# qiaobeibei/PPO-RL-Satellite

Measured on NVIDIA B200. Metric: rk4_env_steps_per_sec, higher is better.
Workload: dtype f64

## Files before the change

### ppo-rl-satellite_b200/build.py

```python
from __future__ import annotations

import os
import subprocess
import sys
from concurrent.futures import ThreadPoolExecutor

HERE = os.path.dirname(os.path.abspath(__file__))
CSRC = os.path.join(HERE, "csrc")
OBJ = os.path.join(HERE, "build")
LIBDIR = os.path.join(HERE, "lib")
LIB = os.path.join(LIBDIR, "libsatb200.so")

ARCH = ["-gencode", "arch=compute_100a,code=sm_100a"]
COMMON = ["-O3", "-lineinfo", "-std=c++17", "-Xcompiler", "-fPIC"]
UNITS = {
    "rk4.cu": ["-fmad=false"],
    "env_step.cu": ["-fmad=false"],
    "gae.cu": ["-fmad=false"],
    "cw_ode.cu": ["-fmad=false"],
    "reach.cu": ["-fmad=false"],
    "actor.cu": [],
    "actor_tc.cu": [],
    "ppo_update.cu": [],
    "ppo_fb_tc.cu": [],
    "ppo_wgrad2_tc.cu": [],
    "capi.cu": [],
}


def _nvcc() -> str:
    for cand in (os.environ.get("NVCC"), "/usr/local/cuda/bin/nvcc", "nvcc"):
        if cand and (os.path.isabs(cand) and os.path.exists(cand) or not os.path.isabs(cand)):
            return cand
    return "nvcc"


def _stale(target: str, deps) -> bool:
    if not os.path.exists(target):
        return True
    t = os.path.getmtime(target)
    return any(os.path.getmtime(d) > t for d in deps)


def build(force: bool = False, verbose: bool = False) -> str:
    os.makedirs(OBJ, exist_ok=True)
    os.makedirs(LIBDIR, exist_ok=True)
    headers = [os.path.join(CSRC, f) for f in os.listdir(CSRC) if f.endswith((".cuh", ".h"))]
    headers.append(os.path.join(os.path.dirname(HERE), "include", "satb200.h"))
    nvcc = _nvcc()
    jobs = []
    objs = []
    for src, extra in UNITS.items():
        s = os.path.join(CSRC, src)
        o = os.path.join(OBJ, src.replace(".cu", ".o"))
        objs.append(o)
        if force or _stale(o, [s] + headers):
            defs = [f"-D{d}" for d in os.environ.get("SAT_NVCC_DEFINES", "").split() if d]
            cmd = [nvcc] + ARCH + COMMON + extra + defs + (["-Xptxas", "-v"] if verbose else []) + ["-c", s, "-o", o]
            jobs.append(cmd)

    def run(cmd):
        r = subprocess.run(cmd, capture_output=True, text=True)
        if r.returncode != 0:
            raise RuntimeError("nvcc failed: %s\n%s\n%s" % (" ".join(cmd), r.stdout, r.stderr))
        if verbose:
            sys.stderr.write(r.stderr)

    with ThreadPoolExecutor(max_workers=min(5, max(1, len(jobs)))) as ex:
        list(ex.map(run, jobs))
    if force or jobs or _stale(LIB, objs):
        run([nvcc] + ARCH + ["-shared", "-o", LIB] + objs + ["-Xcompiler", "-fPIC"])
    return LIB


if __name__ == "__main__":
    print(build(force="--force" in sys.argv, verbose="-v" in sys.argv))
```

### ppo-rl-satellite_b200/csrc/env_step.cu

```cuda
#include "sat_math.cuh"
#include "../../include/satb200.h"
#include <cmath>

namespace {

using namespace sat;

constexpr int kBlock = 128;
constexpr int kEnvsPerBlock = kBlock / 2;
constexpr int kFrontBlock = 64;
#ifndef SAT_FINISH_MINB
#define SAT_FINISH_MINB 7
#endif
constexpr int kFinishMinBlocks = SAT_FINISH_MINB;
constexpr int kObs = 18;
constexpr int kStatDims = 19;
constexpr int kWsHeader = 256;

SAT_DEV double shfl1(double v) { return __shfl_xor_sync(0xffffffffu, v, 1); }
SAT_DEV int shfl1(int v) { return __shfl_xor_sync(0xffffffffu, v, 1); }

SAT_DEV double clip16(double a) { return a < -1.6 ? -1.6 : (a > 1.6 ? 1.6 : a); }

__host__ __device__ inline int64_t ws_disprev_offset() { return kWsHeader; }
__host__ __device__ inline int64_t ws_partials_offset(int64_t n) { return kWsHeader + ((n * 8 + 255) / 256) * 256; }

struct Lane {
    double r[3], v[3];
    double a[3];
    double fuel_own;
    double dis_prev;
};

template <typename ActT>
SAT_DEV void load_and_gate(const SatEnvState& st, const SatEnvParams& p, const ActT* __restrict__ pa,
                           const ActT* __restrict__ ea, int64_t e, int craft, Lane& L, bool do_impulse,
                           const ActT* raw = nullptr ) {
    const int64_t ld = st.ld;
    const double* __restrict__ S = st.state;
    const int32_t* __restrict__ I = st.istate;
    const int base = craft * 6;
#pragma unroll
    for (int k = 0; k < 3; ++k) { L.r[k] = S[(base + k) * ld + e]; L.v[k] = S[(base + 3 + k) * ld + e]; }
    L.fuel_own = S[(SAT_COL_FUEL_C + craft) * ld + e];
    const double dis_stale = S[SAT_COL_DIS * ld + e];
    const int dz_stale = I[SAT_ICOL_DZ * ld + e];
    const int int_state = I[SAT_ICOL_INTSTATE * ld + e];
    {
        const ActT* act = craft ? ea : pa;
#pragma unroll
        for (int k = 0; k < 3; ++k) L.a[k] = clip16((double)(raw ? raw[k] : act[e * 3 + k]));
    }
    bool frozen;
    if (p.flag != 1) frozen = (craft == 0) && (dis_stale < p.d_range) && (dz_stale != 0);
    else frozen = (craft == 1) && (dz_stale == 0);
    if (frozen) { L.a[0] = 0.0; L.a[1] = 0.0; L.a[2] = 0.0; }
    if (!do_impulse) return;
    double d[3];
#pragma unroll
    for (int k = 0; k < 3; ++k) {
        const double o = shfl1(L.r[k]);
        d[k] = craft == 0 ? __dsub_rn(L.r[k], o) : __dsub_rn(o, L.r[k]);
    }
    L.dis_prev = norm3(d);
#pragma unroll
    for (int k = 0; k < 3; ++k) {
        const double s = __dadd_rn(L.v[k], L.a[k]);
        L.v[k] = int_state ? trunc(s) : s;
    }
    L.fuel_own = __dsub_rn(L.fuel_own, __dadd_rn(__dadd_rn(fabs(L.a[0]), fabs(L.a[1])), fabs(L.a[2])));
}

SAT_DEV void propagate_cw(const SatEnvParams& p, Lane& L) {
    const double x6[6] = {L.r[0], L.r[1], L.r[2], L.v[0], L.v[1], L.v[2]};
    double y6[6];
#pragma unroll
    for (int i = 0; i < 6; ++i) y6[i] = gemv6_row(p.stm + 6 * i, x6);
#pragma unroll
    for (int k = 0; k < 3; ++k) { L.r[k] = y6[k]; L.v[k] = y6[3 + k]; }
}

SAT_DEV void propagate_rk4(const SatEnvParams& p, Lane& L) {
    double X[3], V[3];
#pragma unroll
    for (int k = 0; k < 3; ++k) { X[k] = p.r_cw[k] + L.r[k]; V[k] = p.v_cw[k] + L.v[k]; }
    const Rk4Consts c = make_rk4_consts(p.h, p.mu, p.re, p.j2);
    if (p.j2 != 0.0) {
#pragma unroll 1
        for (int s = 0; s < p.substeps; ++s) rk4_step<true>(X, V, c);
    } else {
#pragma unroll 1
        for (int s = 0; s < p.substeps; ++s) rk4_step<false>(X, V, c);
    }
#pragma unroll
    for (int k = 0; k < 3; ++k) { L.r[k] = X[k] - p.r_cw[k]; L.v[k] = V[k] - p.v_cw[k]; }
}

template <typename ActT, bool OBS>
__global__ void __launch_bounds__(kFrontBlock, 14)
env_front_rk4_kernel(const SatEnvState st, const ActT* __restrict__ pa, const ActT* __restrict__ ea,
                     double* __restrict__ dis_prev_out, float* __restrict__ obs_early,
                     float* __restrict__ pa_copy, float* __restrict__ ea_copy, const __grid_constant__ SatEnvParams p) {
    const int64_t tid = (int64_t)blockIdx.x * kFrontBlock + threadIdx.x;
    const int64_t env_raw = tid >> 1;
    const int craft = (int)(tid & 1);
    const bool valid = env_raw < st.n;
    const int64_t e = valid ? env_raw : st.n - 1;
    Lane L;
    if (OBS) {
        ActT raw[3];
        const ActT* act = craft ? ea : pa;
#pragma unroll
        for (int k = 0; k < 3; ++k) raw[k] = act[e * 3 + k];
        if (valid) {
            float* dc = craft ? ea_copy : pa_copy;
#pragma unroll
            for (int k = 0; k < 3; ++k) dc[e * 3 + k] = (float)raw[k];
        }
        load_and_gate(st, p, pa, ea, e, craft, L, true, raw);
    } else {
        load_and_gate(st, p, pa, ea, e, craft, L, true);
    }
    propagate_rk4(p, L);
    if (valid) {
        const int64_t ld = st.ld;
        const int base = craft * 6;
#pragma unroll
        for (int k = 0; k < 3; ++k) { st.state[(base + k) * ld + e] = L.r[k]; st.state[(base + 3 + k) * ld + e] = L.v[k]; }
        st.state[(SAT_COL_FUEL_C + craft) * ld + e] = L.fuel_own;
        if (craft == 0) dis_prev_out[e] = L.dis_prev;
    }
    if (OBS) {
        double P[3], Pv[3], E[3], Ev[3], d[3];
#pragma unroll
        for (int k = 0; k < 3; ++k) {
            const double o_r = shfl1(L.r[k]), o_v = shfl1(L.v[k]);
            P[k] = craft == 0 ? L.r[k] : o_r;  Pv[k] = craft == 0 ? L.v[k] : o_v;
            E[k] = craft == 0 ? o_r : L.r[k];  Ev[k] = craft == 0 ? o_v : L.v[k];
            d[k] = __dsub_rn(P[k], E[k]);
        }
        const double dis = norm3(d);
        const int count_new = st.istate[SAT_ICOL_COUNT * st.ld + e] + 1;
        const bool done = (dis <= p.d_capture) || (count_new >= p.max_episode_steps);
        if (done && p.auto_reset) {
#pragma unroll
            for (int k = 0; k < 3; ++k) { P[k] = p.reset_p[k]; E[k] = p.reset_e[k]; Pv[k] = 0.0; Ev[k] = 0.0; }
        }
        if (valid) {
            float* o = obs_early + e * kObs + craft * 9;
            if (craft == 0) {
#pragma unroll
                for (int k = 0; k < 3; ++k) { o[k] = (float)__dsub_rn(P[k], E[k]); o[3 + k] = (float)__dsub_rn(Pv[k], Ev[k]); o[6 + k] = (float)P[k]; }
            } else {
#pragma unroll
                for (int k = 0; k < 3; ++k) { o[k] = (float)Pv[k]; o[3 + k] = (float)E[k]; o[6 + k] = (float)Ev[k]; }
            }
        }
    }
}

struct SolveQueue {
    double A[2 * kBlock], sth[2 * kBlock], dvm[2 * kBlock], alpha[2 * kBlock];
    int guess[2 * kBlock];
    double trig[2][4];
    int count, next;
};

template <bool EXACT = true>
SAT_DEV void queue_init(SolveQueue& q) {
    if (threadIdx.x == 0) { q.count = 0; q.next = 0; }
    if (threadIdx.x < 4) {
        const int j = threadIdx.x >> 1, k = threadIdx.x & 1;
        const double x0 = dz_guess(j);
        const double h = 1.4901161193847656e-08 * fabs(x0);
        const double2 sc = Lm<EXACT>::sincos(k ? x0 + h : x0);
        q.trig[j][2 * k] = sc.x; q.trig[j][2 * k + 1] = sc.y;
    }
    __syncthreads();
}

SAT_DEV void queue_push(SolveQueue& q, const DzNode& nd, int& slot0, int& slot1, double& alpha0, double& alpha1) {
    slot0 = -1; slot1 = -1; alpha0 = dz_guess(0); alpha1 = dz_guess(1);
    if (nd.status == 2) {
        const bool g0 = dz_degenerate(nd.A0, nd.sth, nd.dvm), g1 = dz_degenerate(nd.A1, nd.sth, nd.dvm);
        const int cnt = (g0 ? 0 : 1) + (g1 ? 0 : 1);
        if (cnt) {
            int s = atomicAdd(&q.count, cnt);
            if (!g0) { slot0 = s; q.A[s] = nd.A0; q.sth[s] = nd.sth; q.dvm[s] = nd.dvm; q.guess[s] = 0; ++s; }
            if (!g1) { slot1 = s; q.A[s] = nd.A1; q.sth[s] = nd.sth; q.dvm[s] = nd.dvm; q.guess[s] = 1; }
        }
    }
    __syncthreads();
}

#ifndef SAT_SOLVE_WARPS
#define SAT_SOLVE_WARPS 4
#endif
template <bool EXACT = true>
SAT_DEV void queue_run(SolveQueue& q) {
    const int total = q.count;
    int task = -1;
    Hybrd1<PFaiT<EXACT>> hs;
    if ((threadIdx.x >> 5) < SAT_SOLVE_WARPS)
    for (;;) {
        if (task < 0) {
            const int t = atomicAdd(&q.next, 1);
            if (t < total) {
                task = t;
                PFaiT<EXACT> f; f.A = q.A[t]; f.sth = q.sth[t]; f.dvm = q.dvm[t];
                hs.init_warm(f, dz_guess(q.guess[t]), q.trig[q.guess[t]]);
            } else task = total;
        }
        const bool active = task < total;
        if (!__any_sync(0xffffffffu, active)) break;
        if (active && hs.step()) { q.alpha[task] = hs.x; task = -1; }
    }
    __syncthreads();
}

template <bool FUSED, typename ActT, int MINB, bool EXACT>
__global__ void __launch_bounds__(kBlock, MINB)
env_step_kernel(const SatEnvState st, const ActT* __restrict__ pa, const ActT* __restrict__ ea,
                const int32_t* __restrict__ count_override, float* __restrict__ obs_f32,
                double* __restrict__ obs_f64, double* __restrict__ term_obs_f64,
                double* __restrict__ reward_out, uint8_t* __restrict__ done_out,
                const double* __restrict__ dis_prev_in, double* __restrict__ partials,
                unsigned int* __restrict__ ticket, const __grid_constant__ SatEnvParams p) {
    union SharedBlock { SolveQueue queue; double tile_term[kEnvsPerBlock][kObs]; __device__ SharedBlock() {} };
    __shared__ SharedBlock shm;
    __shared__ double tile[kEnvsPerBlock][kStatDims];
    SolveQueue& queue = shm.queue;
    double (&tile_term)[kEnvsPerBlock][kObs] = shm.tile_term;
    queue_init<EXACT>(queue);

    const int64_t tid = (int64_t)blockIdx.x * kBlock + threadIdx.x;
    const int64_t env_raw = tid >> 1;
    const int craft = (int)(tid & 1);
    const bool valid = env_raw < st.n;
    const int64_t e = valid ? env_raw : st.n - 1;
    const int64_t ld = st.ld;
    double* __restrict__ S = st.state;
    int32_t* __restrict__ I = st.istate;
    if (ticket && blockIdx.x == 0 && threadIdx.x == 0) *ticket = 0u;

    Lane L;
    load_and_gate(st, p, pa, ea, e, craft, L, FUSED);
    if (FUSED) propagate_cw(p, L);
    else L.dis_prev = dis_prev_in[e];
    const int dz_stale = I[SAT_ICOL_DZ * ld + e];
    const int count = I[SAT_ICOL_COUNT * ld + e];
    int err = I[SAT_ICOL_ERR * ld + e];
    const double ret = S[SAT_COL_RET * ld + e];

    double P[3], Pv[3], E[3], Ev[3], d[3];
#pragma unroll
    for (int k = 0; k < 3; ++k) {
        const double o_r = shfl1(L.r[k]), o_v = shfl1(L.v[k]);
        P[k] = craft == 0 ? L.r[k] : o_r;  Pv[k] = craft == 0 ? L.v[k] : o_v;
        E[k] = craft == 0 ? o_r : L.r[k];  Ev[k] = craft == 0 ? o_v : L.v[k];
        d[k] = __dsub_rn(P[k], E[k]);
    }
    const double dis = norm3(d);
    const int count_new = count_override ? count_override[e] : count + 1;
    const bool captured = dis <= p.d_capture;
    const bool timeout = count_new >= p.max_episode_steps;
    const bool done = captured || timeout;
    const double fuel_oth = shfl1(L.fuel_own);
    const double fuel_c = craft == 0 ? L.fuel_own : fuel_oth;
    double pa_gated[3];
#pragma unroll
    for (int k = 0; k < 3; ++k) { const double o = shfl1(L.a[k]); pa_gated[k] = craft == 0 ? L.a[k] : o; }

    const int le = threadIdx.x >> 1;
    const bool reset_now = done && p.auto_reset;
    const int64_t env0 = (int64_t)blockIdx.x * kEnvsPerBlock;
    const int64_t rem = st.n - env0;
    const int rows = (int)(rem < kEnvsPerBlock ? rem : kEnvsPerBlock);
    {
        double Po[3], Pvo[3], Eo[3], Evo[3];
#pragma unroll
        for (int k = 0; k < 3; ++k) {
            Po[k] = reset_now ? p.reset_p[k] : P[k];  Pvo[k] = reset_now ? 0.0 : Pv[k];
            Eo[k] = reset_now ? p.reset_e[k] : E[k];  Evo[k] = reset_now ? 0.0 : Ev[k];
        }
        if (craft == 0) {
#pragma unroll
            for (int k = 0; k < 3; ++k) { tile[le][k] = __dsub_rn(Po[k], Eo[k]); tile[le][3 + k] = __dsub_rn(Pvo[k], Evo[k]); tile[le][6 + k] = Po[k]; }
        } else {
#pragma unroll
            for (int k = 0; k < 3; ++k) { tile[le][9 + k] = Pvo[k]; tile[le][12 + k] = Eo[k]; tile[le][15 + k] = Evo[k]; }
        }
        __syncthreads();
        const int total = rows * kObs;
        for (int idx = threadIdx.x; idx < total; idx += kBlock) {
            const int row = idx / kObs, col = idx - row * kObs;
            const double val = tile[row][col];
            if (obs_f32) obs_f32[env0 * kObs + idx] = (float)val;
            if (obs_f64) obs_f64[env0 * kObs + idx] = val;
        }
    }

    const bool need_dz = !done && !p.skip_danger_zone && p.flag != 2;
    DzNode nd;
    {
        double Ri[3], Vi[3];
#pragma unroll
        for (int k = 0; k < 3; ++k) { Ri[k] = __dadd_rn(p.r_cw[k], L.r[k]); Vi[k] = __dadd_rn(p.v_cw[k], L.v[k]); }
        dz_prepare<EXACT>(craft, need_dz, Ri, Vi, fuel_c, p.u_grav, nd);
    }
    int slot0, slot1;
    double alpha0, alpha1;
    queue_push(queue, nd, slot0, slot1, alpha0, alpha1);
    queue_run<EXACT>(queue);
    if (slot0 >= 0) alpha0 = queue.alpha[slot0];
    if (slot1 >= 0) alpha1 = queue.alpha[slot1];
    __syncthreads();
    const int dz_eval = dz_finalize<EXACT>(need_dz, nd, alpha0, alpha1, nullptr);
    int dz_new = dz_stale;
    if (need_dz) {
        if (dz_eval >= 0) dz_new = dz_eval;
        else { dz_new = 0; err = 1; }
    }

    double reward = 0.0, cos_a = 0.0, cos_b = 0.0;
    if (p.flag == 2) reward = 0.0;
    else if (captured) reward = (p.flag == 0) ? 100.0 : -150.0;
    else if (timeout) reward = (p.flag == 0) ? 0.0 : 100.0;
    else {
        const bool pv4_on = pa_gated[0] != 0.0 && pa_gated[1] != 0.0 && pa_gated[2] != 0.0;
        double u1[3], w1[3], u2[3], w2[3];
#pragma unroll
        for (int k = 0; k < 3; ++k) {
            u1[k] = craft == 0 ? P[k] : d[k];   w1[k] = craft == 0 ? E[k] : Pv[k];
            u2[k] = craft == 0 ? Pv[k] : d[k];  w2[k] = craft == 0 ? Ev[k] : (pv4_on ? pa_gated[k] : Pv[k]);
        }
// ... 1 lines not shown
        double cb = cosine3(u2, w2);
        if (craft == 1) cb = pv4_on ? -cb : 0.0;
        cos_a = ca; cos_b = cb;
    }
    const double oth_a = shfl1(cos_a), oth_b = shfl1(cos_b);
    if (!captured && !timeout && p.flag != 2) {
        const double pv1 = craft == 0 ? cos_a : oth_a, pv2 = craft == 0 ? cos_b : oth_b;
        const double pv3 = craft == 0 ? oth_a : cos_a, pv4 = craft == 0 ? oth_b : cos_b;
        const double ra = (dis < L.dis_prev) ? 1.0 : -1.0;
        const double rb = (p.d_capture <= dis && dis <= 4.0 * p.d_capture) ? -1.0 : -2.0;
        const double rc = (dz_new == 0) ? -1.0 : dz_new * 0.5;
        double rr = __dadd_rn(__dadd_rn(ra, rb), rc);
        rr = __dadd_rn(rr, pv1);
        rr = __dadd_rn(rr, __dmul_rn(0.6, pv2));
        rr = __dadd_rn(rr, __dmul_rn(0.2, pv3));
        rr = __dadd_rn(rr, __dmul_rn(2.0, pv4));
        reward = (p.flag == 0) ? rr : -rr;
    }
    const double ret_new = __dadd_rn(__dmul_rn(p.gamma, ret), reward);

    if (term_obs_f64) {
        if (craft == 0) {
#pragma unroll
            for (int k = 0; k < 3; ++k) { tile_term[le][k] = d[k]; tile_term[le][3 + k] = __dsub_rn(Pv[k], Ev[k]); tile_term[le][6 + k] = P[k]; }
        } else {
#pragma unroll
            for (int k = 0; k < 3; ++k) { tile_term[le][9 + k] = Pv[k]; tile_term[le][12 + k] = E[k]; tile_term[le][15 + k] = Ev[k]; }
        }
    }

    int int_state_new = 0, count_store = count_new;
    if (reset_now) {
#pragma unroll
        for (int k = 0; k < 3; ++k) {
            P[k] = p.reset_p[k]; E[k] = p.reset_e[k]; Pv[k] = 0.0; Ev[k] = 0.0;
            L.r[k] = craft == 0 ? P[k] : E[k]; L.v[k] = 0.0;
        }
        int_state_new = 1; count_store = 0;
    }

    if (valid) {
        const int base = craft * 6;
        if (FUSED || reset_now) {
#pragma unroll
            for (int k = 0; k < 3; ++k) { S[(base + k) * ld + e] = L.r[k]; S[(base + 3 + k) * ld + e] = L.v[k]; }
        }
        if (FUSED) S[(SAT_COL_FUEL_C + craft) * ld + e] = L.fuel_own;
        if (craft == 0) {
            S[SAT_COL_DIS * ld + e] = dis;
            S[SAT_COL_RET * ld + e] = done ? 0.0 : ret_new;
            I[SAT_ICOL_DZ * ld + e] = dz_new;
            I[SAT_ICOL_COUNT * ld + e] = count_store;
            reward_out[e] = reward;
            done_out[e] = done ? 1 : 0;
        } else {
            I[SAT_ICOL_INTSTATE * ld + e] = int_state_new;
            I[SAT_ICOL_ERR * ld + e] = err;
        }
    }

    if (craft == 0) tile[le][18] = ret_new;
    __syncthreads();
    if (term_obs_f64) {
        const int total = rows * kObs;
        for (int idx = threadIdx.x; idx < total; idx += kBlock) {
            const int row = idx / kObs, col = idx - row * kObs;
            term_obs_f64[env0 * kObs + idx] = tile_term[row][col];
        }
    }
    if (partials && threadIdx.x < kStatDims) {
        const int dim = threadIdx.x;
        double sum = 0.0;
        for (int row = 0; row < rows; ++row) sum += tile[row][dim];
        const double mean = sum / rows;
        double m2 = 0.0;
        for (int row = 0; row < rows; ++row) { double t = tile[row][dim] - mean; m2 += t * t; }
        partials[((int64_t)blockIdx.x * kStatDims + dim) * 2 + 0] = mean;
        partials[((int64_t)blockIdx.x * kStatDims + dim) * 2 + 1] = m2;
    }
}

__global__ void __launch_bounds__(kBlock)
danger_zone_kernel(const double* __restrict__ rv, const double* __restrict__ dv, int64_t n, double u_grav,
                   int32_t* __restrict__ count_out, double* __restrict__ debug_out) {
    __shared__ SolveQueue queue;
    queue_init(queue);
    const int64_t tid = (int64_t)blockIdx.x * kBlock + threadIdx.x;
    const int64_t env_raw = tid >> 1;
    const int craft = (int)(tid & 1);
    const bool valid = env_raw < n;
    const int64_t e = valid ? env_raw : n - 1;
    double Ri[3], Vi[3];
#pragma unroll
    for (int k = 0; k < 3; ++k) { Ri[k] = rv[e * 12 + craft * 6 + k]; Vi[k] = rv[e * 12 + craft * 6 + 3 + k]; }
    DzNode nd;
    dz_prepare(craft, true, Ri, Vi, dv[e], u_grav, nd);
    int slot0, slot1;
    double alpha0, alpha1;
    queue_push(queue, nd, slot0, slot1, alpha0, alpha1);
    queue_run(queue);
    if (slot0 >= 0) alpha0 = queue.alpha[slot0];
    if (slot1 >= 0) alpha1 = queue.alpha[slot1];
    DzDebug dbg = {0, 0, 0, 0, 0, 0, 0, 0};
    const int dz = dz_finalize(true, nd, alpha0, alpha1, debug_out ? &dbg : nullptr);
    if (valid) {
        if (craft == 0) count_out[e] = dz;
        if (debug_out) {
            double* o = debug_out + (e * 2 + craft) * 8;
            o[0] = dbg.rf_max; o[1] = dbg.rf_min; o[2] = dbg.r_ft; o[3] = dbg.alpha0; o[4] = dbg.alpha1;
            o[5] = dbg.theta; o[6] = dbg.dvm; o[7] = dbg.f_cx;
        }
    }
}

__global__ void __launch_bounds__(kBlock)
fsolve_pfai_kernel(const double* __restrict__ dvm, const double* __restrict__ theta, const double* __restrict__ v1x,
                   const double* __restrict__ v1y, const double* __restrict__ h, const double* __restrict__ guess,
                   int64_t n, double u_grav, double* __restrict__ root_out, int32_t* __restrict__ nfev_out) {
    const int64_t i = (int64_t)blockIdx.x * kBlock + threadIdx.x;
    if (i >= n) return;
    double sth, cth;
    glibm::sincos(theta[i], &sth, &cth);
    PFai f;
    f.A = (2.0 * u_grav * (1.0 - cth)) / (h[i] * v1y[i]) - v1x[i] * sth / v1y[i];
    f.sth = sth;
    f.dvm = dvm[i];
    Hybrd1<PFai> hs;
    hs.init(f, guess[i]);
    while (!hs.step()) {}
    root_out[i] = hs.x;
    if (nfev_out) nfev_out[i] = hs.nfev;
}

__global__ void __launch_bounds__(256)
libm_eval_kernel(int fn, const double* __restrict__ x, double* __restrict__ y, int64_t n) {
    const int64_t i = (int64_t)blockIdx.x * 256 + threadIdx.x;
    if (i >= n) return;
    const double v = x[i];
    double r = 0.0, s, c;
    switch (fn) {
        case SAT_LIBM_SIN: r = glibm::sin(v); break;
        case SAT_LIBM_COS: r = glibm::cos(v); break;
        case SAT_LIBM_ACOS: r = glibm::acos(v); break;
        case SAT_LIBM_ATAN: r = glibm::atan(v); break;
        case SAT_LIBM_POW2: r = glibm::pow2(v); break;
        case SAT_LIBM_SINCOS_S: glibm::sincos(v, &s, &c); r = s; break;
        default: glibm::sincos(v, &s, &c); r = c; break;
    }
    y[i] = r;
}

struct Moments { double n, mean, m2; };
SAT_DEV Moments chan(Moments A, Moments B) {
    if (B.n == 0.0) return A;
    if (A.n == 0.0) return B;
    Moments C;
    C.n = A.n + B.n;
    const double delta = B.mean - A.mean;
    C.mean = A.mean + delta * (B.n / C.n);
    C.m2 = A.m2 + B.m2 + delta * delta * (A.n * B.n / C.n);
    return C;
}

SAT_DEV void fold_into_running(double* stats, int dim, int d, Moments B, double* std_out) {
    const double n_old = stats[0];
    const double mean_old = stats[1 + d], S_old = stats[1 + dim + d];
    double n_new, mean_new, S_new, std_new;
    if (B.n == 1.0) {
        const double x = B.mean;
        n_new = n_old + 1.0;
        if (n_new == 1.0) { mean_new = x; S_new = S_old; std_new = x; }
        else {
            mean_new = mean_old + (x - mean_old) / n_new;
            S_new = S_old + (x - mean_old) * (x - mean_new);
            std_new = sqrt(S_new / n_new);
        }
    } else {
        Moments A = {n_old, mean_old, S_old};
        Moments C = chan(A, B);
        n_new = C.n; mean_new = C.mean; S_new = C.m2;
        std_new = sqrt(S_new / n_new);
    }
    stats[1 + d] = mean_new; stats[1 + dim + d] = S_new; stats[1 + 2 * dim + d] = std_new;
    if (std_out) *std_out = std_new;
}

constexpr int kMergeThreads = 256;

SAT_DEV double block_sum_fixed(double v, double* sm) {
#pragma unroll
    for (int off = 16; off > 0; off >>= 1) v += __shfl_xor_sync(0xffffffffu, v, off);
    __syncthreads();
    if ((threadIdx.x & 31) == 0) sm[threadIdx.x >> 5] = v;
    __syncthreads();
    double t = 0.0;
#pragma unroll
    for (int w = 0; w < kMergeThreads / 32; ++w) t += sm[w];
    return t;
}

__global__ void __launch_bounds__(kMergeThreads)
stats_merge_kernel(const double* __restrict__ partials, int64_t nblocks, int64_t n_rows, int rows_per_block,
                   int ndims_in_partials, double* obs_stats, int obs_dim, double* ret_stats, double* ret_std_out,
                   unsigned int* ticket) {
    __shared__ double sm[kMergeThreads / 32];
    const int dim = blockIdx.x;
    const double N = (double)n_rows;
    double wsum = 0.0;
    for (int64_t b = threadIdx.x; b < nblocks; b += kMergeThreads) {
        const int64_t rem = n_rows - b * rows_per_block;
        const double nb = (double)(rem < rows_per_block ? rem : rows_per_block);
        wsum += nb * partials[(b * ndims_in_partials + dim) * 2 + 0];
    }
    const double grand = block_sum_fixed(wsum, sm) / N;
    double m2 = 0.0;
    for (int64_t b = threadIdx.x; b < nblocks; b += kMergeThreads) {
        const int64_t rem = n_rows - b * rows_per_block;
        const double nb = (double)(rem < rows_per_block ? rem : rows_per_block);
        const double dm = partials[(b * ndims_in_partials + dim) * 2 + 0] - grand;
        m2 += partials[(b * ndims_in_partials + dim) * 2 + 1] + nb * dm * dm;
    }
    m2 = block_sum_fixed(m2, sm);
    if (threadIdx.x == 0) {
        Moments B = {N, grand, m2};
        if (dim < obs_dim) { if (obs_stats) fold_into_running(obs_stats, obs_dim, dim, B, nullptr); }
        else if (ret_stats) fold_into_running(ret_stats, 1, 0, B, ret_std_out);
        __threadfence();
        const unsigned int t = atomicAdd(ticket, 1u);
        if (t == gridDim.x - 1) {
            if (obs_stats) obs_stats[0] += N;
            if (ret_stats) ret_stats[0] += N;
            *ticket = 0u;
        }
    }
}

__global__ void env_init_kernel(const SatEnvState st, double fuel_c, double fuel_t,
                                const __grid_constant__ SatEnvParams p, const uint8_t* __restrict__ mask, int full) {
    const int64_t e = (int64_t)blockIdx.x * blockDim.x + threadIdx.x;
    if (e >= st.n) return;
    if (mask && !mask[e]) return;
    const int64_t ld = st.ld;
#pragma unroll
    for (int k = 0; k < 3; ++k) {
        st.state[(SAT_COL_P + k) * ld + e] = p.reset_p[k];
        st.state[(SAT_COL_PV + k) * ld + e] = 0.0;
        st.state[(SAT_COL_E + k) * ld + e] = p.reset_e[k];
        st.state[(SAT_COL_EV + k) * ld + e] = 0.0;
    }
    st.istate[SAT_ICOL_INTSTATE * ld + e] = 1;
    st.istate[SAT_ICOL_COUNT * ld + e] = 0;
    if (full) {
        st.state[SAT_COL_FUEL_C * ld + e] = fuel_c;
        st.state[SAT_COL_FUEL_T * ld + e] = fuel_t;
        st.state[SAT_COL_DIS * ld + e] = INFINITY;
        st.state[SAT_COL_RET * ld + e] = 0.0;
        st.istate[SAT_ICOL_DZ * ld + e] = 0;
        st.istate[SAT_ICOL_ERR * ld + e] = 0;
    }
}

__global__ void env_observe_kernel(const SatEnvState st, float* __restrict__ obs_f32, double* __restrict__ obs_f64) {
    const int64_t idx = (int64_t)blockIdx.x * blockDim.x + threadIdx.x;
    if (idx >= st.n * kObs) return;
    const int64_t e = idx / kObs;
    const int j = (int)(idx - e * kObs);
    const int64_t ld = st.ld;
    const int k = j % 3, g = j / 3;
    double val;
    if (g == 0) val = __dsub_rn(st.state[(SAT_COL_P + k) * ld + e], st.state[(SAT_COL_E + k) * ld + e]);
    else if (g == 1) val = __dsub_rn(st.state[(SAT_COL_PV + k) * ld + e], st.state[(SAT_COL_EV + k) * ld + e]);
    else val = st.state[((g - 2) * 3 + k) * ld + e];
    if (obs_f32) obs_f32[idx] = (float)val;
    if (obs_f64) obs_f64[idx] = val;
}


constexpr int kObsNormEnvs = 128;
__global__ void __launch_bounds__(kObsNormEnvs)
env_observe_norm_kernel(const SatEnvState st, const double* __restrict__ obs_stats, float* __restrict__ obs_f32) {
    __shared__ float tile[kObsNormEnvs * kObs];
    const int64_t e0 = (int64_t)blockIdx.x * kObsNormEnvs;
    const int64_t e = e0 + threadIdx.x;
    const int64_t ld = st.ld;
    if (e < st.n) {
        double P[3], Pv[3], E[3], Ev[3], o[kObs];
#pragma unroll
        for (int k = 0; k < 3; ++k) {
            P[k] = st.state[(SAT_COL_P + k) * ld + e]; Pv[k] = st.state[(SAT_COL_PV + k) * ld + e];
            E[k] = st.state[(SAT_COL_E + k) * ld + e]; Ev[k] = st.state[(SAT_COL_EV + k) * ld + e];
        }
#pragma unroll
        for (int k = 0; k < 3; ++k) {
            o[k] = __dsub_rn(P[k], E[k]); o[3 + k] = __dsub_rn(Pv[k], Ev[k]);
            o[6 + k] = P[k]; o[9 + k] = Pv[k]; o[12 + k] = E[k]; o[15 + k] = Ev[k];
        }
#pragma unroll
        for (int j = 0; j < kObs; ++j) {
            double v = o[j];
            if (obs_stats) v = (v - obs_stats[1 + j]) / (obs_stats[1 + 2 * kObs + j] + 1e-8);
            tile[threadIdx.x * kObs + j] = (float)v;
        }
    }
    __syncthreads();
    const int64_t rem = st.n - e0;
    const int total = (int)(rem < kObsNormEnvs ? rem : kObsNormEnvs) * kObs;
    for (int idx = threadIdx.x; idx < total; idx += kObsNormEnvs) obs_f32[e0 * kObs + idx] = tile[idx];
}

constexpr int kNormRows = 128;

__global__ void __launch_bounds__(kNormRows)
norm_partial_kernel(const double* __restrict__ x, int64_t n, int dim, double* __restrict__ partials,
                    unsigned int* __restrict__ ticket) {
    __shared__ double tile[kNormRows * 32];
    if (blockIdx.x == 0 && threadIdx.x == 0) *ticket = 0u;
    const int64_t row0 = (int64_t)blockIdx.x * kNormRows;
    const int64_t rem = n - row0;
    const int rows = (int)(rem < kNormRows ? rem : kNormRows);
    const int total = rows * dim;
    for (int idx = threadIdx.x; idx < total; idx += kNormRows) tile[idx] = x[row0 * dim + idx];
    __syncthreads();
    if (threadIdx.x < dim) {
        const int d = threadIdx.x;
        double sum = 0.0;
        for (int r = 0; r < rows; ++r) sum += tile[r * dim + d];
        const double mean = sum / rows;
        double m2 = 0.0;
        for (int r = 0; r < rows; ++r) { double t = tile[r * dim + d] - mean; m2 += t * t; }
        partials[((int64_t)blockIdx.x * dim + d) * 2 + 0] = mean;
        partials[((int64_t)blockIdx.x * dim + d) * 2 + 1] = m2;
    }
}

__global__ void norm_apply_kernel(const double* __restrict__ stats, const double* __restrict__ x, int64_t total,
                                  int dim, double* __restrict__ out64, float* __restrict__ out32) {
    const int64_t idx = (int64_t)blockIdx.x * blockDim.x + threadIdx.x;
    if (idx >= total) return;
    const int d = (int)(idx % dim);
    const double mean = stats[1 + d], sd = stats[1 + 2 * dim + d];
    const double y = (x[idx] - mean) / (sd + 1e-8);
    if (out64) out64[idx] = y;
    if (out32) out32[idx] = (float)y;
}

int check_state(const SatEnvState* st) {
    if (!st || !st->state || !st->istate) return SAT_ERR_NULL;
    if (st->n <= 0 || st->ld < st->n || (st->ld & 1)) return SAT_ERR_SIZE;
    if (((uintptr_t)st->state & 15) || ((uintptr_t)st->istate & 15)) return SAT_ERR_SIZE;
    return SAT_OK;
}

inline int launch_status() {
    cudaError_t e = cudaGetLastError();
    return e == cudaSuccess ? SAT_OK : (int)e;
}

}

extern "C" {

int64_t sat_workspace_bytes(int64_t n) {
    if (n <= 0) return kWsHeader;
    int64_t nb_env = (n + kEnvsPerBlock - 1) / kEnvsPerBlock;
    int64_t nb_norm = (n + kNormRows - 1) / kNormRows;
    int64_t a = nb_env * kStatDims * 2 * (int64_t)sizeof(double);
    int64_t b = nb_norm * 32 * 2 * (int64_t)sizeof(double);
    return ws_partials_offset(n) + (a > b ? a : b);
}

void sat_env_default_params(SatEnvParams* p) {
    if (!p) return;
    SatEnvParams q = {};
    q.mode = SAT_MODE_CW; q.flag = 0; q.max_episode_steps = 1000; q.auto_reset = 1;
    q.action_dtype = SAT_ACT_F32; q.substeps = 100; q.skip_danger_zone = 0;
    q.d_capture = 100000.0; q.d_range = 100000.0;
    q.gamma = 0.99;
    q.h = 1.0; q.mu = 3.986e14; q.re = 6378137.0; q.j2 = 0.00108263;
    q.r_cw[0] = 27098000.0; q.r_cw[1] = 32306000.0; q.r_cw[2] = 0.0;
    q.v_cw[0] = -2350.0; q.v_cw[1] = 1970.0; q.v_cw[2] = 0.0;
    q.u_grav = 3.986e14;
    q.reset_p[0] = 200000.0; q.reset_e[0] = 18000.0;
    *p = q;
}

int sat_env_init(const SatEnvState* st, double fuel_c, double fuel_t, const SatEnvParams* p, void* stream) {
    int rc = check_state(st);
    if (rc) return rc;
    if (!p) return SAT_ERR_NULL;
    const int threads = 256;
    const unsigned blocks = (unsigned)((st->n + threads - 1) / threads);
    env_init_kernel<<<blocks, threads, 0, (cudaStream_t)stream>>>(*st, fuel_c, fuel_t, *p, nullptr, 1);
    return launch_status();
}

int sat_env_reset(const SatEnvState* st, const uint8_t* mask, const SatEnvParams* p, void* stream) {
    int rc = check_state(st);
    if (rc) return rc;
    if (!p) return SAT_ERR_NULL;
    const int threads = 256;
    const unsigned blocks = (unsigned)((st->n + threads - 1) / threads);
    env_init_kernel<<<blocks, threads, 0, (cudaStream_t)stream>>>(*st, 0.0, 0.0, *p, mask, 0);
    return launch_status();
}

int sat_env_observe_norm(const SatEnvState* st, const double* obs_stats, float* obs_f32, void* stream) {
    int rc = check_state(st);
    if (rc) return rc;
    if (!obs_f32) return SAT_ERR_NULL;
    const unsigned blocks = (unsigned)((st->n + kObsNormEnvs - 1) / kObsNormEnvs);
    env_observe_norm_kernel<<<blocks, kObsNormEnvs, 0, (cudaStream_t)stream>>>(*st, obs_stats, obs_f32);
    return launch_status();
}

int sat_env_observe(const SatEnvState* st, float* obs_f32, double* obs_f64, void* stream) {
    int rc = check_state(st);
    if (rc) return rc;
    if (!obs_f32 && !obs_f64) return SAT_ERR_NULL;
    const int threads = 256;
    const int64_t total = st->n * kObs;
    const unsigned blocks = (unsigned)((total + threads - 1) / threads);
    env_observe_kernel<<<blocks, threads, 0, (cudaStream_t)stream>>>(*st, obs_f32, obs_f64);
    return launch_status();
}

}

namespace {
int env_step_impl(const SatEnvState* st, const void* pa, const void* ea, const int32_t* count_override,
                  float* obs_f32, double* obs_f64, double* term_obs_f64, double* reward, uint8_t* done,
                  double* obs_stats, double* ret_stats, double* ret_std_out, void* workspace,
                  const SatEnvParams* p, void* stream, cudaEvent_t* ev, float* obs_early = nullptr,
                  cudaEvent_t front_done = nullptr, float* pa_copy = nullptr, float* ea_copy = nullptr) {
    int rc = check_state(st);
    if (rc) return rc;
    if (!pa || !ea || !reward || !done || !p) return SAT_ERR_NULL;
    const bool want_stats = obs_stats || ret_stats;
    if ((want_stats || p->mode == SAT_MODE_RK4) && !workspace) return SAT_ERR_NULL;
    if (p->mode != SAT_MODE_CW && p->mode != SAT_MODE_RK4) return SAT_ERR_MODE;
    if (p->action_dtype != SAT_ACT_F32 && p->action_dtype != SAT_ACT_F64) return SAT_ERR_MODE;
    if (p->flag < 0 || p->flag > 2) return SAT_ERR_MODE;
    if (p->mode == SAT_MODE_RK4 && p->substeps < 1) return SAT_ERR_SIZE;
    if (workspace && ((uintptr_t)workspace & 15)) return SAT_ERR_SIZE;
    cudaStream_t s = (cudaStream_t)stream;
    const int64_t n = st->n;
    const int64_t nblocks = (n + kEnvsPerBlock - 1) / kEnvsPerBlock;
    char* ws = (char*)workspace;
    unsigned int* ticket = ws ? (unsigned int*)ws : nullptr;
    double* dis_prev = ws ? (double*)(ws + ws_disprev_offset()) : nullptr;
    double* partials = want_stats ? (double*)(ws + ws_partials_offset(n)) : nullptr;
    if (ev) cudaEventRecord(ev[0], s);
#define SAT_LAUNCH_FINISH(FUSED, T, ...)                                                                                   \
    do {                                                                                                                   \
        if (p->fast_libm) env_step_kernel<FUSED, T, kFinishMinBlocks, false><<<(unsigned)nblocks, kBlock, 0, s>>>(__VA_ARGS__); \
        else env_step_kernel<FUSED, T, kFinishMinBlocks, true><<<(unsigned)nblocks, kBlock, 0, s>>>(__VA_ARGS__);          \
    } while (0)
    if (p->mode == SAT_MODE_CW) {
        if (ev) cudaEventRecord(ev[1], s);
        if (p->action_dtype == SAT_ACT_F32)
            SAT_LAUNCH_FINISH(true, float, *st, (const float*)pa, (const float*)ea,
                count_override, obs_f32, obs_f64, term_obs_f64, reward, done, nullptr, partials, ticket, *p);
        else
            SAT_LAUNCH_FINISH(true, double, *st, (const double*)pa, (const double*)ea,
                count_override, obs_f32, obs_f64, term_obs_f64, reward, done, nullptr, partials, ticket, *p);
    } else {
        const int64_t fblocks = (2 * n + kFrontBlock - 1) / kFrontBlock;
        if (obs_early && (count_override || p->action_dtype != SAT_ACT_F32 || !pa_copy || !ea_copy)) return SAT_ERR_MODE;
        if (obs_early) {
            env_front_rk4_kernel<float, true><<<(unsigned)fblocks, kFrontBlock, 0, s>>>(*st, (const float*)pa, (const float*)ea,
                                                                                       dis_prev, obs_early, pa_copy, ea_copy, *p);
            if (front_done) cudaEventRecord(front_done, s);
            SAT_LAUNCH_FINISH(false, float, *st, pa_copy, ea_copy,
                count_override, obs_f32, obs_f64, term_obs_f64, reward, done, dis_prev, partials, ticket, *p);
        } else if (p->action_dtype == SAT_ACT_F32) {
            env_front_rk4_kernel<float, false><<<(unsigned)fblocks, kFrontBlock, 0, s>>>(*st, (const float*)pa, (const float*)ea, dis_prev, nullptr, nullptr, nullptr, *p);
            if (ev) cudaEventRecord(ev[1], s);
            SAT_LAUNCH_FINISH(false, float, *st, (const float*)pa, (const float*)ea,
                count_override, obs_f32, obs_f64, term_obs_f64, reward, done, dis_prev, partials, ticket, *p);
        } else {
            env_front_rk4_kernel<double, false><<<(unsigned)fblocks, kFrontBlock, 0, s>>>(*st, (const double*)pa, (const double*)ea, dis_prev, nullptr, nullptr, nullptr, *p);
            if (ev) cudaEventRecord(ev[1], s);
            SAT_LAUNCH_FINISH(false, double, *st, (const double*)pa, (const double*)ea,
                count_override, obs_f32, obs_f64, term_obs_f64, reward, done, dis_prev, partials, ticket, *p);
        }
    }
#undef SAT_LAUNCH_FINISH
    rc = launch_status();
    if (rc) return rc;
    if (ev) cudaEventRecord(ev[2], s);
    if (partials) {
        stats_merge_kernel<<<kStatDims, kMergeThreads, 0, s>>>(partials, nblocks, n, kEnvsPerBlock, kStatDims,
                                                               obs_stats, kObs, ret_stats, ret_std_out, ticket);
        rc = launch_status();
    }
    if (ev) cudaEventRecord(ev[3], s);
    return rc;
}
}

extern "C" {

int sat_env_step(const SatEnvState* st, const void* pa, const void* ea, const int32_t* count_override,
                 float* obs_f32, double* obs_f64, double* term_obs_f64, double* reward, uint8_t* done,
                 double* obs_stats, double* ret_stats, double* ret_std_out, void* workspace,
                 const SatEnvParams* p, void* stream) {
    return env_step_impl(st, pa, ea, count_override, obs_f32, obs_f64, term_obs_f64, reward, done, obs_stats, ret_stats,
                         ret_std_out, workspace, p, stream, nullptr);
}

int sat_env_step_timed(const SatEnvState* st, const void* pa, const void* ea, const int32_t* count_override,
                       float* obs_f32, double* obs_f64, double* term_obs_f64, double* reward, uint8_t* done,
                       double* obs_stats, double* ret_stats, double* ret_std_out, void* workspace,
                       const SatEnvParams* p, void* stream, float* ms_out) {
    if (!ms_out) return SAT_ERR_NULL;
    cudaEvent_t ev[4];
    for (int i = 0; i < 4; ++i) {
        cudaError_t ce = cudaEventCreate(&ev[i]);
        if (ce != cudaSuccess) return (int)ce;
    }
    int rc = env_step_impl(st, pa, ea, count_override, obs_f32, obs_f64, term_obs_f64, reward, done, obs_stats, ret_stats,
                           ret_std_out, workspace, p, stream, ev);
    if (rc == SAT_OK) {
        cudaError_t ce = cudaEventSynchronize(ev[3]);
        if (ce != cudaSuccess) rc = (int)ce;
        else for (int i = 0; i < 3; ++i) cudaEventElapsedTime(&ms_out[i], ev[i], ev[i + 1]);
    }
    for (int i = 0; i < 4; ++i) cudaEventDestroy(ev[i]);
    return rc;
}

int sat_danger_zone_count(const double* rv, const double* dv, int64_t n, double u_grav, int32_t* count_out,
                          double* debug_out, void* stream) {
    if (!rv || !dv || !count_out) return SAT_ERR_NULL;
    if (n <= 0) return SAT_ERR_SIZE;
    const int64_t nblocks = (n + kEnvsPerBlock - 1) / kEnvsPerBlock;
    danger_zone_kernel<<<(unsigned)nblocks, kBlock, 0, (cudaStream_t)stream>>>(rv, dv, n, u_grav, count_out, debug_out);
    return launch_status();
}

int sat_fsolve_pfai(const double* dvm, const double* theta, const double* v1x, const double* v1y, const double* h,
                    const double* guess, int64_t n, double u_grav, double* root_out, int32_t* nfev_out, void* stream) {
    if (!dvm || !theta || !v1x || !v1y || !h || !guess || !root_out) return SAT_ERR_NULL;
    if (n <= 0) return SAT_ERR_SIZE;
    fsolve_pfai_kernel<<<(unsigned)((n + kBlock - 1) / kBlock), kBlock, 0, (cudaStream_t)stream>>>(
        dvm, theta, v1x, v1y, h, guess, n, u_grav, root_out, nfev_out);
    return launch_status();
}

int sat_libm_eval(int fn, const double* x, double* y, int64_t n, void* stream) {
    if (!x || !y) return SAT_ERR_NULL;
    if (n <= 0) return SAT_ERR_SIZE;
    if (fn < SAT_LIBM_SIN || fn > SAT_LIBM_SINCOS_C) return SAT_ERR_MODE;
    libm_eval_kernel<<<(unsigned)((n + 255) / 256), 256, 0, (cudaStream_t)stream>>>(fn, x, y, n);
    return launch_status();
}

int64_t sat_env_step_host_bytes(int64_t n) {
    if (n <= 0) return 0;
    auto al = [](int64_t b) { return (b + 255) / 256 * 256; };
    return al(n * 12) * 2 + al(n * 72) + al(n * 8) + al(n) + sat_workspace_bytes(n) + 16 * sat_workspace_bytes(64) + 16 * 4096;
}

int sat_env_step_host(const SatEnvState* st, const float* pa_host, const float* ea_host,
                      float* obs_host, double* reward_host, uint8_t* done_host, void* d_io,
                      const SatEnvParams* p, void* stream, void* aux_stream, int chunks) {
    int rc = check_state(st);
    if (rc) return rc;
    if (!pa_host || !ea_host || !obs_host || !reward_host || !done_host || !d_io || !p) return SAT_ERR_NULL;
    cudaStream_t s0 = (cudaStream_t)stream, s1 = (cudaStream_t)aux_stream;
    const int64_t n = st->n;
    auto al = [](int64_t b) { return (b + 255) / 256 * 256; };
    char* base = (char*)d_io;
    float* d_pa = (float*)base;
    float* d_ea = (float*)(base + al(n * 12));
    float* d_obs = (float*)(base + 2 * al(n * 12));
    double* d_rew = (double*)(base + 2 * al(n * 12) + al(n * 72));
    uint8_t* d_done = (uint8_t*)(base + 2 * al(n * 12) + al(n * 72) + al(n * 8));
    char* d_ws = base + 2 * al(n * 12) + al(n * 72) + al(n * 8) + al(n);
    SatEnvParams q = *p;
    q.action_dtype = SAT_ACT_F32;
    cudaEvent_t fork = nullptr;
    auto leave = [&](int code) {
        if (fork) {
            cudaStreamSynchronize(s0);
            if (s1) cudaStreamSynchronize(s1);
            cudaEventDestroy(fork);
            fork = nullptr;
        }
        return code;
    };
    if (chunks <= 0) {
        cudaPointerAttributes at;
        bool ok = true;
        const void* ptrs[5] = {pa_host, ea_host, obs_host, reward_host, done_host};
        void* dev[5] = {nullptr, nullptr, nullptr, nullptr, nullptr};
        for (int i = 0; i < 5 && ok; ++i) {
            ok = cudaPointerGetAttributes(&at, ptrs[i]) == cudaSuccess && at.type == cudaMemoryTypeHost && at.devicePointer != nullptr;
            dev[i] = at.devicePointer;
        }
        cudaGetLastError();
        int ranges = (chunks < 0 && s1) ? -chunks : 1;
        if (ranges > 16) ranges = 16;
        if (ok && ranges == 1 && s1 && q.mode == SAT_MODE_RK4) {
            static thread_local cudaEvent_t front_ev[64] = {};
            int devid = 0;
            cudaError_t ce0;
            if ((ce0 = cudaGetDevice(&devid)) != cudaSuccess) return (int)ce0;
            if (devid < 0 || devid >= 64) return SAT_ERR_SIZE;
            cudaEvent_t& fe = front_ev[devid];
            if (!fe && (ce0 = cudaEventCreateWithFlags(&fe, cudaEventDisableTiming)) != cudaSuccess) return (int)ce0;
            rc = env_step_impl(st, dev[0], dev[1], nullptr, nullptr, nullptr, nullptr, (double*)dev[3], (uint8_t*)dev[4],
                               nullptr, nullptr, nullptr, d_ws, &q, (void*)s0, nullptr, d_obs, fe, d_pa, d_ea);
            if (rc) return rc;
            if ((ce0 = cudaStreamWaitEvent(s1, fe, 0)) != cudaSuccess) return (int)ce0;
            if ((ce0 = cudaMemcpyAsync(obs_host, d_obs, (size_t)n * 72, cudaMemcpyDeviceToHost, s1)) != cudaSuccess) return (int)ce0;
            if ((ce0 = cudaStreamSynchronize(s0)) != cudaSuccess) return (int)ce0;
            if ((ce0 = cudaStreamSynchronize(s1)) != cudaSuccess) return (int)ce0;
            return SAT_OK;
        }
// ... 79 lines not shown
```

### ppo-rl-satellite_b200/csrc/sat_math.cuh

```cuda
#pragma once
#include <cstdint>
#include <cuda_runtime.h>
#include "glibm.cuh"

#define SAT_DEV __device__ __forceinline__

namespace sat {

constexpr double kPi = 3.141592653589793;
constexpr double kTwoPi = 2 * 3.141592653589793;

SAT_DEV double dot3(const double a[3], const double b[3]) {
    double s = __dmul_rn(a[0], b[0]);
    s = __fma_rn(a[1], b[1], s);
    s = __fma_rn(a[2], b[2], s);
    return s;
}
SAT_DEV double norm3(const double a[3]) { return __dsqrt_rn(dot3(a, a)); }

SAT_DEV void cross3(const double a[3], const double b[3], double c[3]) {
    c[0] = __dsub_rn(__dmul_rn(a[1], b[2]), __dmul_rn(a[2], b[1]));
    c[1] = __dsub_rn(__dmul_rn(a[2], b[0]), __dmul_rn(a[0], b[2]));
    c[2] = __dsub_rn(__dmul_rn(a[0], b[1]), __dmul_rn(a[1], b[0]));
}

SAT_DEV double gemv6_row(const double* __restrict__ m, const double x[6]) {
    double p0 = __dmul_rn(m[0], x[0]), p1 = __dmul_rn(m[1], x[1]);
    double p2 = __dmul_rn(m[2], x[2]), p3 = __dmul_rn(m[3], x[3]);
    double head = __dadd_rn(__dadd_rn(p0, p2), __dadd_rn(p1, p3));
    double tail = __fma_rn(m[4], x[4], __dmul_rn(m[5], x[5]));
    return __dadd_rn(head, tail);
}

SAT_DEV double cosine3(const double a[3], const double b[3]) {
    double na = norm3(a), nb = norm3(b);
    double ua[3], ub[3];
#pragma unroll
    for (int k = 0; k < 3; ++k) { ua[k] = __ddiv_rn(a[k], na); ub[k] = __ddiv_rn(b[k], nb); }
    return dot3(ua, ub);
}

struct Rk4Consts {
    double h;
    double hh;
    double cx3;
    double cx4;
    double cx1;
    double cv;
    double cj;
};

SAT_DEV Rk4Consts make_rk4_consts(double h, double mu, double re, double j2) {
    Rk4Consts c;
    c.h = h; c.hh = 0.5 * h;
    c.cx3 = -mu * h * h * 0.25; c.cx4 = -mu * h * h * 0.5; c.cx1 = -mu * h * h / 6.0; c.cv = -mu * h / 6.0;
    c.cj = 1.5 * j2 * re * re;
    return c;
}

SAT_DEV double rsqrt_halley(double x) {
    double y0;
    asm("rsqrt.approx.ftz.f64 %0, %1;" : "=d"(y0) : "d"(x));
    double yy = y0 * y0;
    double e = fma(-x, yy, 1.0);
    double p = fma(0.375, e, 0.5);
    double pe = p * e;
    return fma(y0, pe, y0);
}

template <bool J2>
SAT_DEV void accel_scaled(double x, double y, double z, double cj, double& ax, double& ay, double& az) {
    double zz = z * z;
    double r2 = fma(x, x, fma(y, y, zz));
    double ri = rsqrt_halley(r2);
    double ri2 = ri * ri;
    double ri3 = ri2 * ri;
    if (J2) {
        double c = cj * ri2;
        double q = zz * ri2;
        double t1 = fma(-5.0, q, 1.0);
        double g = ri3 * c;
        double kxy = fma(g, t1, ri3);
        double kz = fma(2.0, g, kxy);
        ax = kxy * x; ay = kxy * y; az = kz * z;
    } else {
        ax = ri3 * x; ay = ri3 * y; az = ri3 * z;
    }
}

template <bool J2>
SAT_DEV void rk4_step(double (&x)[3], double (&v)[3], const Rk4Consts& c) {
    double a1[3], a2[3], a3[3], a4[3], xa[3], xb[3], xs[3];
    accel_scaled<J2>(x[0], x[1], x[2], c.cj, a1[0], a1[1], a1[2]);
#pragma unroll
    for (int k = 0; k < 3; ++k) xa[k] = fma(c.hh, v[k], x[k]);
    accel_scaled<J2>(xa[0], xa[1], xa[2], c.cj, a2[0], a2[1], a2[2]);
#pragma unroll
    for (int k = 0; k < 3; ++k) xs[k] = fma(c.cx3, a1[k], xa[k]);
    accel_scaled<J2>(xs[0], xs[1], xs[2], c.cj, a3[0], a3[1], a3[2]);
#pragma unroll
    for (int k = 0; k < 3; ++k) { xb[k] = fma(c.h, v[k], x[k]); xs[k] = fma(c.cx4, a2[k], xb[k]); }
    accel_scaled<J2>(xs[0], xs[1], xs[2], c.cj, a4[0], a4[1], a4[2]);
#pragma unroll
    for (int k = 0; k < 3; ++k) {
        double t = a2[k] + a3[k];
        double s3 = a1[k] + t;
        x[k] = fma(c.cx1, s3, xb[k]);
        double w = (s3 + t) + a4[k];
        v[k] = fma(c.cv, w, v[k]);
    }
}

template <bool EXACT>
struct Lm {
    static SAT_DEV double2 sincos(double x) {
        if (EXACT) return glibm::call::sincos(x);
        double s, c; ::sincos(x, &s, &c); return make_double2(s, c);
    }
    static SAT_DEV double2 sincos_inline(double x) {
        double s, c;
        if (EXACT) glibm::sincos(x, &s, &c); else ::sincos(x, &s, &c);
        return make_double2(s, c);
    }
    static SAT_DEV double cos(double x) { return EXACT ? glibm::call::cos(x) : ::cos(x); }
    static SAT_DEV double acos(double x) { return EXACT ? glibm::call::acos(x) : ::acos(x); }
    static SAT_DEV double atan(double x) { return EXACT ? glibm::call::atan(x) : ::atan(x); }
    static SAT_DEV double pow2(double x) { return EXACT ? glibm::call::pow2(x) : x * x; }
};

struct Elements { double a, e, i, omega, Omega, f; };

template <bool EXACT = true>
SAT_DEV bool orbital_elements(double miu, const double R0[3], const double V0[3], Elements& el) {
    double r_norm = norm3(R0), v_norm = norm3(V0);
    double r_dot_v = dot3(R0, V0);
    double v2 = Lm<EXACT>::pow2(v_norm);
    double energy = 2.0 / r_norm - v2 / miu;
    double c1 = v2 / miu - 1.0 / r_norm, c2 = r_dot_v / miu;
    double E[3], H[3], N[3];
#pragma unroll
    for (int k = 0; k < 3; ++k) E[k] = c1 * R0[k] - c2 * V0[k];
    double e = norm3(E);
    cross3(R0, V0, H);
    double h = norm3(H);
    N[0] = -H[1]; N[1] = H[0]; N[2] = 0.0;
    double n = norm3(N);
    if (energy == 0.0 || e == 0.0) return false;
    el.a = 1.0 / fabs(energy);
    el.e = e;
    el.i = Lm<EXACT>::acos(H[2] / h);
    double omega = (n != 0.0) ? Lm<EXACT>::acos(dot3(N, E) / n / e) : 0.0;
    if (E[2] < 0.0) omega = kTwoPi - omega;
    el.omega = omega;
    double Omega = (n != 0.0) ? Lm<EXACT>::acos(N[0] / n) : 0.0;
    if (N[1] < 0.0) Omega = kTwoPi - Omega;
    el.Omega = Omega;
    double f = Lm<EXACT>::acos(dot3(E, R0) / e / r_norm);
    if (r_dot_v < 0.0) f = kTwoPi - f;
    el.f = f;
    return true;
}

template <bool EXACT>
struct PFaiT {
    double A, sth, dvm;
    SAT_DEV double at(double s, double c) const { return A * (dvm * c) + sth * (-dvm * s); }
// ... 273 lines not shown
```

Before: 331.6 million.

## Add PDL kernel chaining, host-precomputed solver trig, and cheaper J2 acceleration

Launches the env_step and stats-merge kernels with programmatic dependent launch, hoisting independent state loads ahead of griddepcontrol.wait so they overlap the previous kernel's tail. The exact-mode danger-zone trig constants are now computed once on the host and passed as a grid constant instead of evaluated per block on device. The J2 acceleration term is algebraically reordered to save a multiply, which may change f64 rounding relative to the reference.

```diff
diff --git a/ppo-rl-satellite_b200/build.py b/ppo-rl-satellite_b200/build.py
--- a/ppo-rl-satellite_b200/build.py
+++ b/ppo-rl-satellite_b200/build.py
@@ -25,6 +25,7 @@
     "ppo_fb_tc.cu": [],
     "ppo_wgrad2_tc.cu": [],
     "capi.cu": [],
+    "dz_warm.cpp": [],
 }
 
 
@@ -52,7 +53,7 @@
     objs = []
     for src, extra in UNITS.items():
         s = os.path.join(CSRC, src)
-        o = os.path.join(OBJ, src.replace(".cu", ".o"))
+        o = os.path.join(OBJ, os.path.splitext(src)[0] + ".o")
         objs.append(o)
         if force or _stale(o, [s] + headers):
             defs = [f"-D{d}" for d in os.environ.get("SAT_NVCC_DEFINES", "").split() if d]
diff --git a/ppo-rl-satellite_b200/csrc/dz_warm.cpp b/ppo-rl-satellite_b200/csrc/dz_warm.cpp
--- /dev/null
+++ b/ppo-rl-satellite_b200/csrc/dz_warm.cpp
@@ -0,0 +1,15 @@
+#include "glibm.cuh"
+
+namespace sat {
+
+void dz_warm_trig(double trig[2][4]) {
+    const double half_pi = 3.141592653589793 / 2;
+    for (int j = 0; j < 2; ++j) {
+        const double x0 = j == 0 ? half_pi : -half_pi;
+        const double h = glibm::mul_(1.4901161193847656e-08, glibm::abs_(x0));
+        glibm::sincos(x0, &trig[j][0], &trig[j][1]);
+        glibm::sincos(glibm::add_(x0, h), &trig[j][2], &trig[j][3]);
+    }
+}
+
+}
diff --git a/ppo-rl-satellite_b200/csrc/env_step.cu b/ppo-rl-satellite_b200/csrc/env_step.cu
--- a/ppo-rl-satellite_b200/csrc/env_step.cu
+++ b/ppo-rl-satellite_b200/csrc/env_step.cu
@@ -1,6 +1,11 @@
 #include "sat_math.cuh"
 #include "../../include/satb200.h"
 #include <cmath>
+#include <utility>
+
+namespace sat {
+void dz_warm_trig(double trig[2][4]);
+}
 
 namespace {
 
@@ -20,6 +25,9 @@
 SAT_DEV double shfl1(double v) { return __shfl_xor_sync(0xffffffffu, v, 1); }
 SAT_DEV int shfl1(int v) { return __shfl_xor_sync(0xffffffffu, v, 1); }
 
+SAT_DEV void pdl_launch_dependents() { asm volatile("griddepcontrol.launch_dependents;"); }
+SAT_DEV void pdl_wait() { asm volatile("griddepcontrol.wait;" ::: "memory"); }
+
 SAT_DEV double clip16(double a) { return a < -1.6 ? -1.6 : (a > 1.6 ? 1.6 : a); }
 
 __host__ __device__ inline int64_t ws_disprev_offset() { return kWsHeader; }
@@ -101,6 +109,7 @@
 env_front_rk4_kernel(const SatEnvState st, const ActT* __restrict__ pa, const ActT* __restrict__ ea,
                      double* __restrict__ dis_prev_out, float* __restrict__ obs_early,
                      float* __restrict__ pa_copy, float* __restrict__ ea_copy, const __grid_constant__ SatEnvParams p) {
+    pdl_launch_dependents();
     const int64_t tid = (int64_t)blockIdx.x * kFrontBlock + threadIdx.x;
     const int64_t env_raw = tid >> 1;
     const int craft = (int)(tid & 1);
@@ -166,14 +175,25 @@
     int count, next;
 };
 
+struct DzWarm { double trig[2][4]; };
+
+DzWarm dz_warm_exact() {
+    static const DzWarm w = [] { DzWarm t; sat::dz_warm_trig(t.trig); return t; }();
+    return w;
+}
+
 template <bool EXACT = true>
-SAT_DEV void queue_init(SolveQueue& q) {
+SAT_DEV void queue_init(SolveQueue& q, const DzWarm& w) {
     if (threadIdx.x == 0) { q.count = 0; q.next = 0; }
     if (threadIdx.x < 4) {
         const int j = threadIdx.x >> 1, k = threadIdx.x & 1;
-        const double x0 = dz_guess(j);
-        const double h = 1.4901161193847656e-08 * fabs(x0);
-        const double2 sc = Lm<EXACT>::sincos(k ? x0 + h : x0);
+        double2 sc;
+        if (EXACT) sc = make_double2(w.trig[j][2 * k], w.trig[j][2 * k + 1]);
+        else {
+            const double x0 = dz_guess(j);
+            const double h = 1.4901161193847656e-08 * fabs(x0);
+            sc = Lm<EXACT>::sincos(k ? x0 + h : x0);
+        }
         q.trig[j][2 * k] = sc.x; q.trig[j][2 * k + 1] = sc.y;
     }
     __syncthreads();
@@ -225,13 +245,15 @@
                 double* __restrict__ obs_f64, double* __restrict__ term_obs_f64,
                 double* __restrict__ reward_out, uint8_t* __restrict__ done_out,
                 const double* __restrict__ dis_prev_in, double* __restrict__ partials,
-                unsigned int* __restrict__ ticket, const __grid_constant__ SatEnvParams p) {
+                unsigned int* __restrict__ ticket, const __grid_constant__ SatEnvParams p,
+                const __grid_constant__ DzWarm warm) {
+    pdl_launch_dependents();
     union SharedBlock { SolveQueue queue; double tile_term[kEnvsPerBlock][kObs]; __device__ SharedBlock() {} };
     __shared__ SharedBlock shm;
     __shared__ double tile[kEnvsPerBlock][kStatDims];
     SolveQueue& queue = shm.queue;
     double (&tile_term)[kEnvsPerBlock][kObs] = shm.tile_term;
-    queue_init<EXACT>(queue);
+    queue_init<EXACT>(queue, warm);
 
     const int64_t tid = (int64_t)blockIdx.x * kBlock + threadIdx.x;
     const int64_t env_raw = tid >> 1;
@@ -242,15 +264,16 @@
     double* __restrict__ S = st.state;
     int32_t* __restrict__ I = st.istate;
     if (ticket && blockIdx.x == 0 && threadIdx.x == 0) *ticket = 0u;
-
+    const int dz_stale = I[SAT_ICOL_DZ * ld + e];
+    const int count = I[SAT_ICOL_COUNT * ld + e];
+    int err = I[SAT_ICOL_ERR * ld + e];
+    const double ret = S[SAT_COL_RET * ld + e];
+
+    pdl_wait();
     Lane L;
     load_and_gate(st, p, pa, ea, e, craft, L, FUSED);
     if (FUSED) propagate_cw(p, L);
     else L.dis_prev = dis_prev_in[e];
-    const int dz_stale = I[SAT_ICOL_DZ * ld + e];
-    const int count = I[SAT_ICOL_COUNT * ld + e];
-    int err = I[SAT_ICOL_ERR * ld + e];
-    const double ret = S[SAT_COL_RET * ld + e];
 
     double P[3], Pv[3], E[3], Ev[3], d[3];
 #pragma unroll
@@ -418,9 +441,9 @@
 
 __global__ void __launch_bounds__(kBlock)
 danger_zone_kernel(const double* __restrict__ rv, const double* __restrict__ dv, int64_t n, double u_grav,
-                   int32_t* __restrict__ count_out, double* __restrict__ debug_out) {
+                   int32_t* __restrict__ count_out, double* __restrict__ debug_out, const __grid_constant__ DzWarm warm) {
     __shared__ SolveQueue queue;
-    queue_init(queue);
+    queue_init(queue, warm);
     const int64_t tid = (int64_t)blockIdx.x * kBlock + threadIdx.x;
     const int64_t env_raw = tid >> 1;
     const int craft = (int)(tid & 1);
@@ -540,6 +563,7 @@
                    int ndims_in_partials, double* obs_stats, int obs_dim, double* ret_stats, double* ret_std_out,
                    unsigned int* ticket) {
     __shared__ double sm[kMergeThreads / 32];
+    pdl_wait();
     const int dim = blockIdx.x;
     const double N = (double)n_rows;
     double wsum = 0.0;
@@ -689,6 +713,18 @@
 
 inline int launch_status() {
     cudaError_t e = cudaGetLastError();
+    return e == cudaSuccess ? SAT_OK : (int)e;
+}
+
+template <typename... KArgs, typename... Args>
+int launch(bool pdl, void (*kernel)(KArgs...), unsigned grid, unsigned block, cudaStream_t s, Args&&... args) {
+    cudaLaunchConfig_t cfg = {};
+    cfg.gridDim = dim3(grid); cfg.blockDim = dim3(block); cfg.stream = s;
+    cudaLaunchAttribute attr[1];
+    attr[0].id = cudaLaunchAttributeProgrammaticStreamSerialization;
+    attr[0].val.programmaticStreamSerializationAllowed = 1;
+    cfg.attrs = attr; cfg.numAttrs = pdl ? 1 : 0;
+    const cudaError_t e = cudaLaunchKernelEx(&cfg, kernel, std::forward<Args>(args)...);
     return e == cudaSuccess ? SAT_OK : (int)e;
 }
 
@@ -785,11 +821,15 @@
     unsigned int* ticket = ws ? (unsigned int*)ws : nullptr;
     double* dis_prev = ws ? (double*)(ws + ws_disprev_offset()) : nullptr;
     double* partials = want_stats ? (double*)(ws + ws_partials_offset(n)) : nullptr;
+    const DzWarm warm = dz_warm_exact();
+    const bool chain = !ev;
     if (ev) cudaEventRecord(ev[0], s);
 #define SAT_LAUNCH_FINISH(FUSED, T, ...)                                                                                   \
     do {                                                                                                                   \
-        if (p->fast_libm) env_step_kernel<FUSED, T, kFinishMinBlocks, false><<<(unsigned)nblocks, kBlock, 0, s>>>(__VA_ARGS__); \
-        else env_step_kernel<FUSED, T, kFinishMinBlocks, true><<<(unsigned)nblocks, kBlock, 0, s>>>(__VA_ARGS__);          \
+        rc = launch(!FUSED && chain && !front_done, p->fast_libm ? env_step_kernel<FUSED, T, kFinishMinBlocks, false>                              \
+                                         : env_step_kernel<FUSED, T, kFinishMinBlocks, true>,                              \
+                    (unsigned)nblocks, kBlock, s, __VA_ARGS__, warm);                                                      \
+        if (rc) return rc;                                                                                                 \
     } while (0)
     if (p->mode == SAT_MODE_CW) {
         if (ev) cudaEventRecord(ev[1], s);
@@ -825,9 +865,9 @@
     if (rc) return rc;
     if (ev) cudaEventRecord(ev[2], s);
     if (partials) {
-        stats_merge_kernel<<<kStatDims, kMergeThreads, 0, s>>>(partials, nblocks, n, kEnvsPerBlock, kStatDims,
-                                                               obs_stats, kObs, ret_stats, ret_std_out, ticket);
-        rc = launch_status();
+        rc = launch(chain, stats_merge_kernel, kStatDims, kMergeThreads, s, partials, nblocks, n, kEnvsPerBlock, kStatDims,
+                    obs_stats, kObs, ret_stats, ret_std_out, ticket);
+        if (rc == SAT_OK) rc = launch_status();
     }
     if (ev) cudaEventRecord(ev[3], s);
     return rc;
@@ -870,7 +910,8 @@
     if (!rv || !dv || !count_out) return SAT_ERR_NULL;
     if (n <= 0) return SAT_ERR_SIZE;
     const int64_t nblocks = (n + kEnvsPerBlock - 1) / kEnvsPerBlock;
-    danger_zone_kernel<<<(unsigned)nblocks, kBlock, 0, (cudaStream_t)stream>>>(rv, dv, n, u_grav, count_out, debug_out);
+    danger_zone_kernel<<<(unsigned)nblocks, kBlock, 0, (cudaStream_t)stream>>>(rv, dv, n, u_grav, count_out, debug_out,
+                                                                               dz_warm_exact());
     return launch_status();
 }
 
diff --git a/ppo-rl-satellite_b200/csrc/sat_math.cuh b/ppo-rl-satellite_b200/csrc/sat_math.cuh
--- a/ppo-rl-satellite_b200/csrc/sat_math.cuh
+++ b/ppo-rl-satellite_b200/csrc/sat_math.cuh
@@ -76,12 +76,10 @@
     double ri2 = ri * ri;
     double ri3 = ri2 * ri;
     if (J2) {
-        double c = cj * ri2;
-        double q = zz * ri2;
-        double t1 = fma(-5.0, q, 1.0);
-        double g = ri3 * c;
-        double kxy = fma(g, t1, ri3);
-        double kz = fma(2.0, g, kxy);
+        double ri5 = ri3 * ri2;
+        double w = fma(-5.0 * cj * zz, ri2, cj);
+        double kxy = fma(ri5, w, ri3);
+        double kz = fma(2.0 * cj, ri5, kxy);
         ax = kxy * x; ay = kxy * y; az = kz * z;
     } else {
         ax = ri3 * x; ay = ri3 * y; az = ri3 * z;
```

Result: faster. 338.6 million, median of 6 (+2.1%).
